# nijaru/sy

Hardware: AMD Instinct MI355X
Metric: GiB/s device-resident delta signature+match, 4 KiB blocks; % HBM-read peak (higher is better)
Workload: dtype u8

## Files before the change

### sy_amd/csrc/sydelta_kernels.hip

```cpp
#include "sydelta_device.hpp"
#include "sydelta_internal.hpp"
#include "sydelta_zstdbatch.hpp"

#include <hipcub/hipcub.hpp>

#include <algorithm>
#include <chrono>
#include <mutex>

namespace sydelta {

#include "sydelta_kcommon.hpp"


__global__ __launch_bounds__(256) void k_sig_fast(const uint8_t* __restrict__ buf, uint64_t nfull, uint32_t bs,
                                                  uint32_t* __restrict__ weak, uint64_t* __restrict__ strong) {
    const uint32_t lane = threadIdx.x & 63;
    const uint64_t blk = ((((uint64_t)blockIdx.x * blockDim.x + threadIdx.x) >> 6) << 2) + (lane >> 4);
    if ((blk & ~3ull) >= nfull) return;
    const bool live = blk < nfull;
    uint32_t wk;
    uint64_t st;
    row_hash(buf + (live ? blk : (nfull - 1)) * (uint64_t)bs, bs, wk, st);
    if ((lane & 15) == 0 && live) {
// ... 962 lines not shown
                si = cur->seg_id;
                if (p < cur->pos_end) {
                    slot = table_find(cur->keys, cur->bmask, ew);
                    fslot = (uint32_t)cur->slot_off;
                }
                rp = (uint32_t)(p - cur->pos_begin);
            } else {
                const uint32_t t = t_begin + (ex >> 14);
                si = seg_of_tile(a, t);
                const ScanSeg S = a.segs[si];
                const uint64_t p = S.pos_begin + (uint64_t)(t - S.tile_base) * kTile2 + (ex & (kTile2 - 1));
                if (p < S.pos_end) {
                    const FileIx F = a.files[S.file];
                    slot = table_find(a.keys + F.slot_off, F.bmask, ew);
                    fslot = (uint32_t)F.slot_off;
                }
                rp = (uint32_t)(p - S.pos_begin);
            }
        }
        const bool hit = slot >= 0;
        const uint64_t m = __ballot(hit);
        if (!m) continue;
        const uint32_t cnt = __popcll(m);
        weak_hits += cnt;
        if (nwq + cnt > (uint32_t)kWQ2) {
            lds_fence();
            verify3<kRowVerify>(a, wq, nwq, rows, tile_start, cur);
            nwq = 0;
        }
        if (hit) wq[nwq + __popcll(m & ((1ull << lane) - 1))] = make_uint4(si, rp, fslot + (uint32_t)slot, 0);
        nwq += cnt;
    }
    lds_fence();
    if (tw) { const unsigned long long t1 = __builtin_amdgcn_s_memtime(); t_lk += t1 - t0; t0 = t1; }
    verify3<kRowVerify>(a, wq, nwq, rows, tile_start, cur);
    lds_fence();
    if (tw) {
        t_vf += __builtin_amdgcn_s_memtime() - t0;
        atomicAdd(&a.counters[8], t_lk);
        atomicAdd(&a.counters[9], t_vf);
    }
}

template <bool kLdsFilter, int kWgPerCu = kLdsFilter ? 3 : 4, bool kRowVerify = false>
__global__ __launch_bounds__(kT2, kWgPerCu) void k_scan_lds(ScanArgs a, uint32_t per, uint32_t lds_fwords) {
    constexpr bool kTileFlush = !kLdsFilter;
    extern __shared__ __attribute__((aligned(16))) unsigned char smem[];
    const uint32_t n = a.n;
    const Lds2 L = lds2_layout(n, kLdsFilter ? lds_fwords : 0u);
    uint32_t* rows = (uint32_t*)smem;
    uint32_t* PS = (uint32_t*)(smem + L.ps);
    uint32_t* PV = (uint32_t*)(smem + L.pv);
    uint64_t* PJ = (uint64_t*)(smem + L.pj);
    uint32_t* ntab = (uint32_t*)(smem + L.ntab);
    uint32_t* lfilt = (uint32_t*)(smem + L.filt);
    const uint32_t tid = threadIdx.x;
    const uint32_t lane = tid & 63, wid = tid >> 6;
    uint4* wq = (uint4*)(smem + L.q) + (size_t)wid * kWQ2;
    uint2* fq = a.gfq + ((size_t)blockIdx.x * (kT2 / 64) + wid) * kGFQ;
    __shared__ uint32_t red_s[kT2 / 64], red_v[kT2 / 64];
    __shared__ uint64_t red_j[kT2 / 64];

    const uint32_t t_begin = blockIdx.x * per;
    const uint32_t t_end = min(a.ntiles, t_begin + per);
    if (t_begin >= t_end) return;
    const uint32_t nch = L.nch;

    for (uint32_t i = tid; i < 256; i += kT2) ntab[i] = kMod - 1 - (a.nm * i) % kMod;
    const uint32_t sh = n & 3;
    const uint32_t rel0 = tid * kR2;
    unsigned long long passes = 0, weak_hits = 0;
    uint32_t nfq = 0;
    uint32_t cur_file = 0xFFFFFFFFu;
    uint32_t fwshift = 0;
    const uint32_t* gfilt = a.filt;
    SegCtx sc;

    unsigned long long tm[4] = {0, 0, 0, 0};
    unsigned long long tprev = a.timing ? __builtin_amdgcn_s_memtime() : 0;
#define PHASE_MARK(k)                                                  \
    if (a.timing) {                                                    \
        const unsigned long long tnow = __builtin_amdgcn_s_memtime(); \
        tm[k] += tnow - tprev;                                         \
        tprev = tnow;                                                  \
    }
    uint32_t si = 0;
#pragma unroll 1
    for (uint32_t tile = t_begin; tile < t_end; ++tile) {
        if (tile == t_begin || (si + 1 < a.nsegs && a.segs[si + 1].tile_base <= tile)) {
            uint32_t lo = si, hi = a.nsegs;
            if (tile == t_begin) lo = 0;
            while (hi - lo > 1) {
                const uint32_t mid = (lo + hi) >> 1;
                if (a.segs[mid].tile_base <= tile) lo = mid; else hi = mid;
            }
            si = lo;
            const ScanSeg S = a.segs[si];
            const FileIx F = a.files[S.file];
            sc.base = a.src + S.src;
            sc.pos_begin = S.pos_begin;
            sc.pos_end = S.pos_end;
            sc.keys = a.keys + F.slot_off;
            sc.slot_off = F.slot_off;
            sc.bmask = F.bmask;
            sc.seg_id = si;
            fwshift = F.fwshift;
            gfilt = a.filt + F.filt_off;
            if (kLdsFilter && S.file != cur_file) {
                const uint4* src4 = (const uint4*)gfilt;
                uint4* dst4 = (uint4*)lfilt;
                const uint32_t fwords = 1u << (32 - fwshift);
#pragma unroll 4
                for (uint32_t i = tid; i < fwords / 4; i += kT2) dst4[i] = src4[i];
            }
            cur_file = S.file;
        }
        const uint64_t seg_len = a.segs[si].len;
        const uint64_t tile_start = sc.pos_begin + (uint64_t)(tile - a.segs[si].tile_base) * kTile2;

#pragma unroll 1
        for (uint32_t c = tid; c < nch; c += kT2) {
            uint32_t x[16];
            load_chunk_nt(sc.base, seg_len, tile_start + 64ull * c, x);
            uint32_t S = 0, V = 0;
#pragma unroll
            for (int i = 0; i < 16; ++i) {
                S = udot4(x[i], 0x01010101u, S);
                V = udot4(x[i], offw(i), V);
                rows[c * kRowDw + i] = x[i];
            }
            PS[c] = S;
            PV[c] = V;
        }
        __syncthreads();
        PHASE_MARK(0)

        {
            const uint32_t per_t = (nch + kT2 - 1) / kT2;
            const uint32_t c_lo = min(nch, tid * per_t), c_hi = min(nch, c_lo + per_t);
            uint32_t ts = 0, tv = 0;
            uint64_t tj = 0;
            for (uint32_t c = c_lo; c < c_hi; ++c) { ts += PS[c]; tv += PV[c]; tj += (uint64_t)c * PS[c]; }
            uint32_t is = ts, iv = tv;
            uint64_t ij = tj;
#pragma unroll
            for (int m = 1; m < 64; m <<= 1) {
                const uint32_t os = (uint32_t)__shfl_up((int)is, m, 64);
                const uint32_t ov = (uint32_t)__shfl_up((int)iv, m, 64);
                const uint32_t ojl = (uint32_t)__shfl_up((int)(uint32_t)ij, m, 64);
                const uint32_t ojh = (uint32_t)__shfl_up((int)(uint32_t)(ij >> 32), m, 64);
                if (lane >= (uint32_t)m) { is += os; iv += ov; ij += ((uint64_t)ojh << 32) | ojl; }
            }
            if (lane == 63) { red_s[wid] = is; red_v[wid] = iv; red_j[wid] = ij; }
            __syncthreads();
            uint32_t bs_ = 0, bv_ = 0;
            uint64_t bj_ = 0;
            for (uint32_t w = 0; w < wid; ++w) { bs_ += red_s[w]; bv_ += red_v[w]; bj_ += red_j[w]; }
            uint32_t es = bs_ + is - ts, ev = bv_ + iv - tv;
            uint64_t ej = bj_ + ij - tj;
            for (uint32_t c = c_lo; c < c_hi; ++c) {
                const uint32_t s0 = PS[c], v0 = PV[c];
                PS[c] = es; PV[c] = ev; PJ[c] = ej;
                es += s0; ev += v0; ej += (uint64_t)c * s0;
            }
            if (tid == kT2 - 1) { PS[nch] = bs_ + is; PV[nch] = bv_ + iv; PJ[nch] = bj_ + ij; }
            __syncthreads();
        }

        uint32_t am, bm;
        {
            const uint32_t c0 = tid, m = n >> 6, rem = n & 63;
            const uint64_t dS = PS[c0 + m] - PS[c0];
            const uint64_t dV = PV[c0 + m] - PV[c0];
            const uint64_t dJ = PJ[c0 + m] - PJ[c0];
            uint64_t A = dS;
            uint64_t B = (uint64_t)n * dS - 64ull * (dJ - (uint64_t)c0 * dS) - dV;
            for (uint32_t r = 0; r < rem; ++r) {
                const uint32_t xr = (rows[(c0 + m) * kRowDw + (r >> 2)] >> (8 * (r & 3))) & 0xFF;
                A += xr;
                B += (uint64_t)(rem - r) * xr;
            }
            am = (uint32_t)((1 + A) % kMod);
            bm = (uint32_t)((n + B) % kMod);
        }
        PHASE_MARK(1)

        const uint32_t qtile = (tile - t_begin) << 14;
#pragma unroll 1
        for (uint32_t g = 0; g < (uint32_t)kR2; g += kB2) {
            if (nfq > (uint32_t)(kGFQ - 64 * kB2)) {
                passes += nfq;
                drain3<kRowVerify>(a, fq, nfq, wq, t_begin, weak_hits, kTileFlush ? rows : nullptr, tile_start,
                       kTileFlush ? &sc : nullptr);
                nfq = 0;
            }
            uint32_t xo[4], xi[4];
#pragma unroll
            for (int j = 0; j < 4; ++j) xo[j] = rows[tid * kRowDw + (g >> 2) + j];
            {
                const uint32_t d0 = (rel0 + g + n) >> 2;
                uint32_t dw[5];
#pragma unroll
                for (int j = 0; j < 5; ++j) {
                    const uint32_t d = d0 + j;
                    dw[j] = rows[(d >> 4) * kRowDw + (d & 15)];
                }
#pragma unroll
                for (int j = 0; j < 4; ++j) xi[j] = __builtin_amdgcn_alignbyte(dw[j + 1], dw[j], sh);
            }
            uint32_t ct[kB2];
#pragma unroll
            for (int t = 0; t < kB2; ++t) ct[t] = ntab[(xo[t >> 2] >> (8 * (t & 3))) & 0xFF];
            uint32_t wv[kB2], fh[kB2], fw[kB2];
#pragma unroll
            for (int t = 0; t < kB2; ++t) {
                const uint32_t out = (xo[t >> 2] >> (8 * (t & 3))) & 0xFF;
                const uint32_t in = (xi[t >> 2] >> (8 * (t & 3))) & 0xFF;
                wv[t] = (bm << 16) | am;
                const ProbeHash h = probe_hash(am, bm);
                fh[t] = h.q;
                fw[t] = kLdsFilter ? lfilt[h.r >> fwshift] : gfilt[h.r >> fwshift];
                uint32_t u = am + in - out;
                u = min(u, u + kMod);
                am = min(u, u - kMod);
                uint32_t v = bm + am + ct[t];
                v = min(v, v - kMod);
                bm = min(v, v - kMod);
            }
#pragma unroll
            for (int t = 0; t < kB2; ++t) {
                const bool pass = filt_pass(fw[t], fh[t]);
                const uint64_t mk = __ballot(pass);
                if (mk) {
                    if (pass) fq[nfq + __popcll(mk & ((1ull << lane) - 1))] = make_uint2(qtile | (rel0 + g + t), wv[t]);
                    nfq += __popcll(mk);
                }
            }
        }
        PHASE_MARK(2)
        if (kTileFlush && nfq) {
            passes += nfq;
            drain3<kRowVerify>(a, fq, nfq, wq, t_begin, weak_hits, rows, tile_start, &sc);
            nfq = 0;
        }
        __syncthreads();
        PHASE_MARK(3)
    }
    passes += nfq;
    drain3<kRowVerify>(a, fq, nfq, wq, t_begin, weak_hits);
#undef PHASE_MARK
    if (lane == 0 && passes) atomicAdd(&a.counters[2], passes);
    if (lane == 0 && weak_hits) atomicAdd(&a.counters[1], weak_hits);
    if (a.timing && tid == 0)
        for (int k = 0; k < 4; ++k) atomicAdd(&a.counters[4 + k], tm[k]);
}

constexpr int kB3 = 8;
constexpr uint32_t kMaxN3 = 4096;
constexpr uint32_t kMulti = 0x80000000u;

__device__ __forceinline__ bool fat_find_k(const uint32_t* __restrict__ keys, const uint4* __restrict__ fat,
                                           uint32_t bmask, uint32_t w, uint4& rec) {
    uint32_t b = bucket_hash(w) & bmask;
    for (;;) {
        const uint4 k = *(const uint4*)(keys + 4 * (size_t)b);
        const int j = k.x == w ? 0 : k.y == w ? 1 : k.z == w ? 2 : k.w == w ? 3 : -1;
        if (j >= 0) {
            rec = fat[4 * (size_t)b + j];
            return true;
        }
        if (k.w == kEmptyKey) return false;
        b = (b + 1) & bmask;
    }
}


struct L1Batch {
    uint32_t w2[kB3], hq[kB3], wv[kB3];
};

__device__ __forceinline__ void load16_nt(const uint8_t* src, uint64_t len, uint64_t c0, uint32_t x[4]) {
    if (c0 + 16 <= len) {
        const uint4* q = (const uint4*)(src + c0);
        x[0] = __builtin_nontemporal_load(&q->x);
        x[1] = __builtin_nontemporal_load(&q->y);
        x[2] = __builtin_nontemporal_load(&q->z);
        x[3] = __builtin_nontemporal_load(&q->w);
    } else {
#pragma unroll
        for (int i = 0; i < 4; ++i) {
            uint32_t v = 0;
            for (int b = 0; b < 4; ++b) {
                const uint64_t p = c0 + 4 * i + b;
                if (p < len) v |= (uint32_t)src[p] << (8 * b);
            }
            x[i] = v;
        }
    }
}

constexpr int kTR = 512;
constexpr int kWTR = 4096;
constexpr int kNBR = 64 / kB3;
static_assert(kMaxN3 == 4096 && kWTR % kMaxN3 == 0, "k_scan_r: a lane's in row is row l of the next wave tile");

struct LdsR {
    uint32_t l1, ntab, kt, ctr, total;
};
__host__ __device__ constexpr LdsR ldsr_layout() {
    LdsR L{};
    uint32_t o = 0;
    L.l1 = o; o += kL1WordsR * 4;
    L.ntab = o; o += 256 * 4;
    L.kt = o; o += 48 * 8;
    L.ctr = o; o += 16;
    L.total = o;
    return L;
}
static_assert(ldsr_layout().total <= 160 * 1024 - 256, "k_scan_r's LDS");

constexpr int kKtW = 0, kKtLast = 24, kKtInit = 32, kKtMerge = 40, kKtWords = 48;
typedef uint32_t v16u32 __attribute__((ext_vector_type(16)));

__device__ __forceinline__ uint64_t dpp64_ctrl_shr4(uint64_t v) {
    return ((uint64_t)dpp32<0x114>((uint32_t)(v >> 32)) << 32) | dpp32<0x114>((uint32_t)v);
}
__device__ __forceinline__ uint64_t dpp64_ctrl_shl4(uint64_t v) {
    return ((uint64_t)dpp32<0x104>((uint32_t)(v >> 32)) << 32) | dpp32<0x104>((uint32_t)v);
}
template <int kCtrl>
__device__ __forceinline__ uint64_t dpp64(uint64_t v) {
    return ((uint64_t)dpp32<kCtrl>((uint32_t)(v >> 32)) << 32) | dpp32<kCtrl>((uint32_t)v);
}

__device__ __forceinline__ uint64_t wave_strong_regs(const uint32_t (&xo)[16], const uint32_t (&xi)[16], uint32_t o,
                                                  const uint64_t* kt) {
    const uint32_t lane = threadIdx.x & 63;
    o = __builtin_amdgcn_readfirstlane(o);
    const uint32_t lp = o >> 6, c = o & 63, q = c >> 2, sh = c & 3;
    v16u32 S0, S1;
#pragma unroll
    for (int r = 0; r < 16; ++r) {
        S0[r] = lane >= lp ? xo[r] : xi[r];
        S1[r] = lane > lp ? xo[r] : xi[r];
    }
    const int addrA = (int)(((lp + lane) & 63) << 2), addrB = (int)(((lp + lane + 1) & 63) << 2);
    uint32_t raw[17];
#pragma unroll
    for (int j = 0; j < 17; ++j) {
        const uint32_t r = q + j;
        const uint32_t v = r < 16 ? S0[r & 15] : S1[r & 15];
        raw[j] = (uint32_t)__builtin_amdgcn_ds_bpermute(r < 16 ? addrA : addrB, (int)v);
    }
    const uint32_t kb = lane == 63 ? (uint32_t)kKtLast : (lane & 15);
    uint64_t cc[8];
#pragma unroll
    for (int i = 0; i < 8; ++i) cc[i] = 0;
#pragma unroll
    for (int i = 0; i < 8; ++i) {
        const uint32_t w0 = __builtin_amdgcn_alignbyte(raw[2 * i + 1], raw[2 * i], sh);
        const uint32_t w1 = __builtin_amdgcn_alignbyte(raw[2 * i + 2], raw[2 * i + 1], sh);
        const uint64_t v = (uint64_t)w0 | ((uint64_t)w1 << 32);
        const uint64_t dk = v ^ kt[kb + i];
        cc[i ^ 1] += v;
        cc[i] += mul32x32(dk);
    }
    uint64_t f;
    const bool b3 = lane & 8, b2 = lane & 4, b1 = lane & 2;
    uint64_t d[4], e[2];
#pragma unroll
    for (int k = 0; k < 4; ++k) {
        const uint64_t send = b3 ? cc[k] : cc[4 + k], keep = b3 ? cc[4 + k] : cc[k];
        d[k] = keep + dpp64<kDppRowRor8>(send);
    }
#pragma unroll
    for (int k = 0; k < 2; ++k) {
        const uint64_t send = b2 ? d[k] : d[2 + k], keep = b2 ? d[2 + k] : d[k];
        const uint64_t from_lo = dpp64_ctrl_shr4(send), from_hi = dpp64_ctrl_shl4(send);
        e[k] = keep + (b2 ? from_lo : from_hi);
    }
    {
        const uint64_t send = b1 ? e[0] : e[1], keep = b1 ? e[1] : e[0];
        f = keep + dpp64<kDppQuadXor2>(send);
    }
    f += dpp64<kDppQuadXor1>(f);
    const uint64_t p1 = shfl64(f, (int)((lane + 16) & 63));
    const uint64_t p2 = shfl64(f, (int)((lane + 32) & 63));
    const uint64_t p3 = shfl64(f, (int)((lane + 48) & 63));
    const uint32_t ai = (lane >> 1) & 7;
    const uint64_t skey = kt[kKtW + 16 + ai];
    uint64_t acc = kt[kKtInit + ai] + f;
    acc = scramble1(acc, skey) + p1;
    acc = scramble1(acc, skey) + p2;
    acc = scramble1(acc, skey) + p3;
    const uint64_t z = acc ^ kt[kKtMerge + ai];
    const uint64_t zp = dpp64<kDppQuadXor2>(z);
    uint64_t m = (lane & 3) == 0 ? fold64(z, zp) : 0ull;
    m += dpp64<kDppRowRor4>(m);
    m += dpp64<kDppRowRor8>(m);
    const uint64_t h = xxh3_aval((uint64_t)4096 * P64_1 + m);
    return ((uint64_t)__builtin_amdgcn_readlane((int)(uint32_t)(h >> 32), 0) << 32) |
           (uint32_t)__builtin_amdgcn_readlane((int)(uint32_t)h, 0);
}

constexpr uint32_t kHStage = 256;
constexpr uint32_t kDStage = 64;

struct WaveOut {
    uint4* h;
    WDef* d;
    uint32_t nh;
    uint32_t nd;
};

__device__ __forceinline__ WaveOut wave_out(const ScanArgs& a, uint64_t gwave) {
    WaveOut o;
    o.h = a.hstage + gwave * kHStage;
    o.d = a.dstage ? a.dstage + gwave * kDStage : nullptr;
    o.nh = 0;
    o.nd = 0;
    return o;
}

__device__ __forceinline__ void flush_hits(const ScanArgs& a, WaveOut& o) {
    if (!o.nh) return;
    const uint32_t lane = threadIdx.x & 63;
    __threadfence_block();
    unsigned long long k0 = 0;
    if (lane == 0) k0 = atomicAdd(&a.counters[0], (unsigned long long)o.nh);
    k0 = shfl64(k0, 0);
    for (uint32_t i = lane; i < o.nh; i += 64) {
        const volatile uint4* g = o.h + i;
        const uint32_t lo = g->x, hi = g->y, blk = g->z;
        const unsigned long long k = k0 + i;
        if (k < a.out_cap) {
            a.hit_key[k] = ((uint64_t)hi << 32) | lo;
            a.hit_val[k] = blk;
        }
    }
    o.nh = 0;
}

__device__ __forceinline__ void stage_hits(const ScanArgs& a, WaveOut& o, bool v, uint64_t key, uint32_t blk) {
    const uint64_t m = __ballot(v);
    if (!m) return;
    const uint32_t c = __popcll(m);
    if (o.nh + c > kHStage) flush_hits(a, o);
    const uint32_t lane = threadIdx.x & 63;
    if (v) o.h[o.nh + __popcll(m & ((1ull << lane) - 1))] = make_uint4((uint32_t)key, (uint32_t)(key >> 32), blk, 0);
    o.nh += c;
}

__device__ __forceinline__ uint32_t verify_def(const ScanArgs& a, const WDef& d) {
    uint64_t st;
    if (a.n > 240) {
        uint32_t wk;
        wave_hash_long(a.src + d.at, a.n, wk, st);
    } else {
        st = 0;
        if ((threadIdx.x & 63) == 0) st = xxh3_short(a.src + d.at, a.n);
        st = shfl64(st, 0);
    }
    if (!(d.cand & kMulti)) return st == d.strong ? d.cand : kNoBlock;
    return first_strong_match(a.order, a.cstrong, a.start[d.cand & ~kMulti], a.cnt[d.cand & ~kMulti], st);
}

__device__ __forceinline__ void flush_defs(const ScanArgs& a, WaveOut& o) {
    if (!o.nd) return;
    const uint32_t lane = threadIdx.x & 63;
    __threadfence_block();
    unsigned long long k0 = 0;
    if (lane == 0) k0 = atomicAdd(&a.counters[10], (unsigned long long)o.nd);
    k0 = shfl64(k0, 0);
    for (uint32_t i = lane; i < o.nd; i += 64) {
        const unsigned long long k = k0 + i;
        if (k < a.wdef_cap) {
            const volatile uint64_t* g = (const volatile uint64_t*)(o.d + i);
            WDef d;
            d.at = g[0];
            d.key = g[1];
            const uint64_t cp = g[2];
            d.cand = (uint32_t)cp;
            d.pad = 0;
            d.strong = g[3];
            a.wdef[k] = d;
        }
    }
    if (k0 + o.nd > a.wdef_cap) {
        const uint32_t first = k0 >= a.wdef_cap ? 0u : (uint32_t)(a.wdef_cap - k0);
        for (uint32_t i = first; i < o.nd; ++i) {
            const volatile uint64_t* g = (const volatile uint64_t*)(o.d + i);
            WDef d;
            d.at = g[0];
            d.key = g[1];
            d.cand = (uint32_t)g[2];
            d.pad = 0;
            d.strong = g[3];
            const uint32_t best = verify_def(a, d);
            stage_hits(a, o, lane == 0 && best != kNoBlock, d.key, best);
        }
    }
    o.nd = 0;
}

__device__ __forceinline__ void stage_defs(const ScanArgs& a, WaveOut& o, bool v, const WDef& d) {
    const uint64_t m = __ballot(v);
    if (!m) return;
    const uint32_t c = __popcll(m);
    if (o.nd + c > kDStage) flush_defs(a, o);
    const uint32_t lane = threadIdx.x & 63;
    if (v) o.d[o.nd + __popcll(m & ((1ull << lane) - 1))] = d;
    o.nd += c;
}

template <bool kSmall = false>
__device__ __forceinline__ void drain_regs(const ScanArgs& a, const uint2* recs, uint32_t nr, uint32_t tile_rel,
                                           const uint32_t (&xo)[16], const uint32_t (&xi)[16], const uint64_t* kt,
                                           unsigned long long& weak_hits, uint64_t run_start, const SegCtx& cur,
                                           WaveOut& o) {
    const uint32_t lane = threadIdx.x & 63;
    __threadfence_block();
    for (uint32_t base = 0; base < nr; base += 64) {
        const uint32_t i = base + lane;
        bool hit = false;
        uint4 rec = make_uint4(0, 0, 0, 0);
        uint32_t pos = 0;
        if (i < nr) {
            const volatile uint2* g = recs + i;
            pos = g->x;
            const uint32_t w = g->y;
            if (run_start + pos < cur.pos_end) {
                if (kSmall) {
                    const int64_t sl = table_find(cur.keys, cur.bmask, w);
                    hit = sl >= 0;
                    rec.y = kMulti | (uint32_t)(cur.slot_off + (uint64_t)(sl < 0 ? 0 : sl));
                } else {
                    hit = fat_find_k(cur.keys, cur.fat, cur.bmask, w, rec);
                }
            }
        }
        uint64_t m = __ballot(hit);
        weak_hits += __popcll(m);
        uint32_t best_mine = kNoBlock;
        while (m) {
            const int h = __builtin_ctzll(m);
            m &= m - 1;
            const uint32_t hp = __builtin_amdgcn_readlane((int)pos, h);
            const uint32_t hy = __builtin_amdgcn_readlane((int)rec.y, h);
            const uint64_t hs = ((uint64_t)(uint32_t)__builtin_amdgcn_readlane((int)rec.w, h) << 32) |
                                (uint32_t)__builtin_amdgcn_readlane((int)rec.z, h);
            const uint64_t st = wave_strong_regs(xo, xi, hp - tile_rel, kt);
            uint32_t best = kNoBlock;
            if (!(hy & kMulti)) {
                if (st == hs) best = hy;
            } else {
                best = first_strong_match(a.order, a.cstrong, a.start[hy & ~kMulti], a.cnt[hy & ~kMulti], st);
            }
            if ((int)lane == h) best_mine = best;
        }
        stage_hits(a, o, best_mine != kNoBlock,
                   ((uint64_t)cur.seg_id << kSegShift) | (uint64_t)(run_start + pos - cur.pos_begin), best_mine);
    }
}

template <bool kRib, int kWaves, bool kSmall = false>
__global__ __launch_bounds__(kWaves * 64, 1) void k_scan_r(ScanArgs a, uint32_t per, uint32_t small_words) {
    extern __shared__ __attribute__((aligned(16))) unsigned char smem[];
    constexpr LdsR L = ldsr_layout();
    constexpr uint32_t kT = kWaves * 64;
    const uint32_t n = a.n;
    const uint32_t* l1 = (const uint32_t*)(smem + L.l1);
    uint32_t* ntab = (uint32_t*)(smem + L.ntab);
    const uint32_t tid = threadIdx.x;
    const uint32_t lane = tid & 63, wid = tid >> 6;
    uint32_t* ctr = (uint32_t*)(smem + L.ctr);
    const uint32_t gwave = blockIdx.x * kWaves + wid;
    uint2* rec = a.rrec + (size_t)gwave * kWTR;
    uint32_t* fslot = (uint32_t*)(smem + L.l1) + (size_t)wid * small_words;
    uint32_t slot_file = 0xFFFFFFFFu;
    WaveOut wo = wave_out(a, gwave);

    const uint32_t t_begin = blockIdx.x * per;
    const uint32_t t_end = min(a.ntiles, t_begin + per);
    if (t_begin >= t_end) return;
    if (!kSmall) {
        const uint4* g = (const uint4*)a.l1;
        uint4* d = (uint4*)(smem + L.l1);
#pragma unroll 4
        for (uint32_t i = tid; i < kL1WordsR / 4; i += kT) d[i] = g[i];
    }
    for (uint32_t i = tid; i < 256; i += kT) ntab[i] = kMod - 1 - (a.nm * i) % kMod;
    uint64_t* kt = (uint64_t*)(smem + L.kt);
    if (tid < 48)
        kt[tid] = tid < 24 ? c_tab.w[tid] : tid < 32 ? c_tab.last[tid - 24] : tid < 40 ? c_tab.init[tid - 32]
                                                                                       : c_tab.merge[tid - 40];
    if (tid == 0) *ctr = 0;
    __syncthreads();

    unsigned long long passes = 0, weak_hits = 0;
    uint32_t nrec = 0, si_hint = 0;
    const uint64_t below = (1ull << lane) - 1;
#pragma unroll 1
    for (;;) {
        uint32_t c = 0;
        if (lane == 0) c = atomicAdd(ctr, 1u);
        c = __builtin_amdgcn_readfirstlane(c);
        const uint32_t t0 = t_begin + 2 * c;
        if (t0 >= t_end) break;
        const uint32_t tz = min(t_end, t0 + 2);
#pragma unroll 1
        for (uint32_t t = t0; t < tz;) {
            uint32_t lo = si_hint, hi = a.nsegs;
            while (hi - lo > 1) {
                const uint32_t mid = (lo + hi) >> 1;
                if (a.segs[mid].tile_base <= t) lo = mid; else hi = mid;
            }
            const uint32_t si = lo;
            si_hint = si;
            const ScanSeg S = a.segs[si];
            const FileIx F = a.files[S.file];
            SegCtx sc;
            sc.base = a.src + S.src;
            sc.pos_begin = S.pos_begin;
            sc.keys = a.keys + F.slot_off;
            sc.fat = a.fat + F.slot_off;
            sc.slot_off = F.slot_off;
            sc.bmask = F.bmask;
            sc.seg_id = si;
            sc.fwshift = F.fwshift;
            sc.filt = a.filt + F.filt_off;
            sc.fwords = 1u << (32 - F.fwshift);
            const uint32_t span = (t + 1 < tz && !(si + 1 < a.nsegs && a.segs[si + 1].tile_base <= t + 1)) ? 2u : 1u;
            const uint64_t run_start = S.pos_begin + (uint64_t)(t - S.tile_base) * kTile2;
            sc.pos_end = min(S.pos_end, run_start + (uint64_t)span * kTile2);
            const uint64_t seg_len = S.len;
            const uint32_t nwt = span * (kTile2 / kWTR);
            t += span;

            const uint64_t fptr = (uint64_t)(uintptr_t)sc.filt;
            const uint32_t fp_lo = __builtin_amdgcn_readfirstlane((uint32_t)fptr);
            const uint32_t fp_hi = __builtin_amdgcn_readfirstlane((uint32_t)(fptr >> 32));
            const __amdgpu_buffer_rsrc_t frsrc = __builtin_amdgcn_make_buffer_rsrc(
                (void*)(uintptr_t)(((uint64_t)fp_hi << 32) | fp_lo), (short)0,
                (int)__builtin_amdgcn_readfirstlane(sc.fwords * 4), 0x00020000);
            const uint32_t fwshift = __builtin_amdgcn_readfirstlane(sc.fwshift);
            if (kSmall && S.file != slot_file) {
                slot_file = S.file;
                lds_fence();
                const uint4* g = (const uint4*)sc.filt;
                uint4* d = (uint4*)fslot;
                for (uint32_t i = lane; i < sc.fwords / 4; i += 64) d[i] = g[i];
                lds_fence();
            }

            uint32_t xo[16], xi[16], xn[16];
            load_chunk_nt(sc.base, seg_len, run_start + 64ull * lane, xo);
            load_chunk_nt(sc.base, seg_len, run_start + n + 64ull * lane, xi);
#pragma unroll 1
            for (uint32_t k = 0; k < nwt; ++k) {
                const uint64_t P = run_start + (uint64_t)k * kWTR;
                const uint32_t rel0 = k * kWTR + lane * 64;
                uint32_t am, bm;
                {
                    uint32_t Sx[2], Vx[2], Jx[2], TS[2], TV[2], TJ[2];
#pragma unroll
                    for (int j = 0; j < 2; ++j) {
                        uint32_t s = 0, v = 0;
#pragma unroll
                        for (int i = 0; i < 16; ++i) {
                            const uint32_t d = j ? xi[i] : xo[i];
                            s = udot4(d, 0x01010101u, s);
                            v = udot4(d, offw(i), v);
                        }
                        Sx[j] = wave_scan_excl(s, TS[j]);
                        Vx[j] = wave_scan_excl(v, TV[j]);
                        Jx[j] = wave_scan_excl((uint32_t)(64 * j + lane) * s, TJ[j]);
                    }
                    const uint64_t dS = TS[0] + Sx[1] - Sx[0];
                    const uint64_t dV = TV[0] + Vx[1] - Vx[0];
                    const uint64_t dJ = TJ[0] + Jx[1] - Jx[0];
                    const uint32_t A = (uint32_t)dS;
                    const uint32_t B = (uint32_t)((uint64_t)n * dS - 64ull * (dJ - (uint64_t)lane * dS) - dV);
                    am = (1 + A) % kMod;
                    bm = (n + B) % kMod;
                }
                auto compute = [&](const int g, L1Batch& Bt) {
                    const uint32_t xo0 = xo[g >> 2], xo1 = xo[(g >> 2) + 1];
                    const uint32_t xi0 = xi[g >> 2], xi1 = xi[(g >> 2) + 1];
                    uint32_t ct[kB3], rr[kB3], w1[kB3], w1b[kB3], bo[kB3];
#pragma unroll
                    for (int t2 = 0; t2 < kB3; ++t2) ct[t2] = ntab[((t2 < 4 ? xo0 : xo1) >> (8 * (t2 & 3))) & 0xFF];
#pragma unroll
                    for (int t2 = 0; t2 < kB3; ++t2) {
                        const uint32_t out = ((t2 < 4 ? xo0 : xo1) >> (8 * (t2 & 3))) & 0xFF;
                        const uint32_t in = ((t2 < 4 ? xi0 : xi1) >> (8 * (t2 & 3))) & 0xFF;
                        __builtin_assume(am < kMod);
                        __builtin_assume(bm < kMod);
                        Bt.wv[t2] = (bm << 16) | am;
                        const ProbeHash h = probe_hash(am, bm);
                        Bt.hq[t2] = h.q;
                        rr[t2] = h.r;
                        if (kSmall) {
                            Bt.w2[t2] = fslot[h.r >> fwshift];
                        } else if (kRib) {
                            bo[t2] = rib_bit(h.q, h.r);
                            w1[t2] = l1[bo[t2] >> 5];
                            w1b[t2] = l1[(bo[t2] >> 5) + 1];
                        } else {
                            w1[t2] = l1[l1r_word(h.q)];
                        }
                        const uint32_t u = am + in + (kMod - out);
                        am = min(u, min(u - kMod, u - 2 * kMod));
                        const uint32_t v = bm + am + ct[t2];
                        bm = min(v, min(v - kMod, v - 2 * kMod));
                    }
#pragma unroll
                    for (int t2 = 0; t2 < kB3 && !kSmall; ++t2) {
                        uint32_t p1;
                        if (kRib) {
                            const uint32_t win = __builtin_amdgcn_alignbit(w1b[t2], w1[t2], bo[t2]);
                            p1 = ~__builtin_popcount(win & rib_coef(Bt.hq[t2], rr[t2])) & 1u;
                        } else {
                            p1 = l1_test(w1[t2], Bt.hq[t2]);
                        }
                        Bt.w2[t2] = __builtin_amdgcn_raw_buffer_load_b32(frsrc, (int)(((rr[t2] >> fwshift) << 2) | (p1 - 1u)),
                                                                         0, 0);
                    }
                };
                auto finish = [&](const int g, L1Batch& Bt) {
                    uint32_t pbits = 0;
#pragma unroll
                    for (int t2 = 0; t2 < kB3; ++t2) pbits |= filt_bit(Bt.w2[t2], Bt.hq[t2]) << t2;
                    asm volatile("" : "+v"(pbits));
                    if (!__ballot(pbits != 0)) return;
#pragma unroll
                    for (int t2 = 0; t2 < kB3; ++t2) {
                        const uint64_t mk = __ballot((pbits >> t2) & 1);
                        if (!mk) continue;
                        if ((pbits >> t2) & 1) rec[nrec + __popcll(mk & below)] = make_uint2(rel0 + g + t2, Bt.wv[t2]);
                        nrec += __popcll(mk);
                    }
                };
                const uint32_t tile_rec = nrec;
                L1Batch b0, b1;
                compute(0, b0);
                compute(8, b1);
#pragma unroll
                for (int bi = 0; bi < kNBR; ++bi) {
                    L1Batch& Bt = (bi & 1) ? b1 : b0;
                    finish(kB3 * bi, Bt);
                    if (bi + 2 < kNBR) compute(kB3 * (bi + 2), Bt);
                    if (bi == 2 && k + 1 < nwt)
                        load_chunk_nt(sc.base, seg_len, P + n + kWTR + 64ull * lane, xn);
                }
                passes += nrec - tile_rec;
                if (nrec > tile_rec)
                    drain_regs<kSmall>(a, rec + tile_rec, nrec - tile_rec, k * kWTR, xo, xi, kt, weak_hits, run_start, sc,
                                       wo);
                nrec = tile_rec;
#pragma unroll
                for (int i = 0; i < 16; ++i) {
                    xo[i] = xi[i];
                    xi[i] = xn[i];
                }
            }
        }
    }
    flush_hits(a, wo);
    if (lane == 0 && passes) atomicAdd(&a.counters[2], passes);
    if (lane == 0 && weak_hits) atomicAdd(&a.counters[1], weak_hits);
}


__device__ __forceinline__ void load64_u(const uint8_t* src, uint64_t len, uint64_t q, uint32_t x[16]) {
    const uint32_t sh = (uint32_t)q & 15u;
    if (!sh) {
        load_chunk(src, len, q, x);
        return;
    }
    const uint64_t qa = q - sh;
    const uint4* g = (const uint4*)(src + qa);
    uint32_t d[20];
    if (qa + 80 <= len) {
#pragma unroll
        for (int i = 0; i < 5; ++i) {
            const uint4 v = g[i];
            d[4 * i] = v.x; d[4 * i + 1] = v.y; d[4 * i + 2] = v.z; d[4 * i + 3] = v.w;
        }
    } else {
#pragma unroll
        for (int i = 0; i < 5; ++i) {
            uint4 v = make_uint4(0, 0, 0, 0);
            if (qa + 16 * i < len) v = g[i];
            d[4 * i] = v.x; d[4 * i + 1] = v.y; d[4 * i + 2] = v.z; d[4 * i + 3] = v.w;
        }
#pragma unroll
        for (int i = 0; i < 20; ++i) {
            const uint64_t o = qa + 4 * i;
            d[i] &= o >= len ? 0u : (o + 4 <= len ? 0xFFFFFFFFu : (0xFFFFFFFFu >> (8 * (o + 4 - len))));
        }
    }
    const uint32_t ds = sh >> 2, bs = sh & 3;
    uint32_t e[17];
#pragma unroll
    for (int i = 0; i < 17; ++i) e[i] = ds == 0 ? d[i] : ds == 1 ? d[i + 1] : ds == 2 ? d[i + 2] : d[i + 3];
#pragma unroll
    for (int i = 0; i < 16; ++i) x[i] = __builtin_amdgcn_alignbyte(e[i + 1], e[i], bs);
}

__device__ __forceinline__ void window_at(const uint8_t* src, uint64_t len, uint64_t P, uint32_t n, uint32_t& am,
                                          uint32_t& bm) {
    const uint32_t lane = threadIdx.x & 63;
    uint64_t s = 0, t = 0;
    for (uint32_t c = 64 * lane; c < n; c += 64 * 64) {
        uint32_t x[16];
        load64_u(src, len, P + c, x);
        uint32_t cs = 0, cv = 0;
#pragma unroll
        for (int i = 0; i < 16; ++i) {
            const uint32_t j = c + 4 * i;
            const uint32_t keep = j >= n ? 0u : (j + 4 <= n ? 0xFFFFFFFFu : (0xFFFFFFFFu >> (8 * (j + 4 - n))));
            const uint32_t v = x[i] & keep;
            cs = udot4(v, 0x01010101u, cs);
            cv = udot4(v, offw(i), cv);
        }
        s += cs;
        t += (uint64_t)c * cs + cv;
    }
    s = wave_sum64(s);
    t = wave_sum64(t);
    am = (uint32_t)((1 + s) % kMod);
    bm = (uint32_t)((n + (uint64_t)n * s - t) % kMod);
}

__device__ __forceinline__ void drain_g(const ScanArgs& a, const uint2* recs, uint32_t nr, unsigned long long& weak_hits,
                                        uint64_t run_start, const SegCtx& cur, WaveOut& o) {
    const uint32_t lane = threadIdx.x & 63;
    __threadfence_block();
    for (uint32_t base = 0; base < nr; base += 64) {
        const uint32_t i = base + lane;
        bool hit = false;
        uint4 rec = make_uint4(0, 0, 0, 0);
        uint32_t pos = 0;
        if (i < nr) {
            const volatile uint2* g = recs + i;
            pos = g->x;
            const uint32_t w = g->y;
            if (run_start + pos < cur.pos_end) hit = fat_find_k(cur.keys, cur.fat, cur.bmask, w, rec);
        }
        const uint64_t m = __ballot(hit);
        if (!m) continue;
        weak_hits += __popcll(m);
        const uint64_t p = run_start + pos;
        WDef d;
        d.at = (uint64_t)(cur.base - a.src) + p;
        d.key = ((uint64_t)cur.seg_id << kSegShift) | (p - cur.pos_begin);
        d.cand = rec.y;
        d.pad = 0;
        d.strong = ((uint64_t)rec.w << 32) | rec.z;
        stage_defs(a, o, hit, d);
    }
}

__device__ __forceinline__ void drain_gs(const ScanArgs& a, const uint2* recs, uint32_t nr,
                                         unsigned long long& weak_hits, uint64_t run_start, const SegCtx& cur,
                                         WaveOut& o) {
    const uint32_t lane = threadIdx.x & 63;
    __threadfence_block();
    for (uint32_t base = 0; base < nr; base += 64) {
        const uint32_t i = base + lane;
        bool hit = false;
        uint32_t pos = 0, gslot = 0;
        if (i < nr) {
            const volatile uint2* g = recs + i;
            pos = g->x;
            const uint32_t w = g->y;
            if (run_start + pos < cur.pos_end) {
                const int64_t sl = table_find(cur.keys, cur.bmask, w);
                hit = sl >= 0;
                gslot = (uint32_t)(cur.slot_off + (uint64_t)(sl < 0 ? 0 : sl));
            }
        }
        const uint64_t m = __ballot(hit);
        if (!m) continue;
        weak_hits += __popcll(m);
        const uint64_t p = run_start + pos;
        WDef d;
        d.at = (uint64_t)(cur.base - a.src) + p;
        d.key = ((uint64_t)cur.seg_id << kSegShift) | (p - cur.pos_begin);
        d.cand = kMulti | gslot;
        d.pad = 0;
        d.strong = 0;
        stage_defs(a, o, hit, d);
    }
}

struct LdsG {
    uint32_t l1, ntab, ctr, total;
};
__host__ __device__ constexpr LdsG ldsg_layout(uint32_t small_words = 0) {
    LdsG L{};
    uint32_t o = 0;
    L.l1 = o; o += small_words ? (kTR / 64) * small_words * 4 : kL1WordsR * 4;
    L.ntab = o; o += 256 * 4;
    L.ctr = o; o += 16;
    L.total = o;
    return L;
}
static_assert(ldsg_layout().total <= 160 * 1024 - 256, "k_scan_g's LDS");

template <bool kRib, bool kSmall>
__global__ __launch_bounds__(kTR, 2) void k_scan_g(ScanArgs a, uint32_t per, uint32_t rt, uint32_t small_words) {
    extern __shared__ __attribute__((aligned(16))) unsigned char smem[];
    const LdsG L = ldsg_layout(kSmall ? small_words : 0u);
    const uint32_t n = a.n;
    const uint32_t* l1 = (const uint32_t*)(smem + L.l1);
    uint32_t* ntab = (uint32_t*)(smem + L.ntab);
    const uint32_t tid = threadIdx.x;
    const uint32_t lane = tid & 63, wid = tid >> 6;
    uint32_t* ctr = (uint32_t*)(smem + L.ctr);
    const uint32_t gwave = blockIdx.x * (kTR / 64) + wid;
    uint2* rec = a.rrec + (size_t)gwave * kWTR;
    WaveOut wo = wave_out(a, gwave);
    uint32_t* fslot = (uint32_t*)(smem + L.l1) + (size_t)wid * small_words;

    const uint32_t t_begin = blockIdx.x * per;
    const uint32_t t_end = min(a.ntiles, t_begin + per);
    if (t_begin >= t_end) return;
    if (!kSmall) {
        const uint4* g = (const uint4*)a.l1;
        uint4* d = (uint4*)(smem + L.l1);
#pragma unroll 4
        for (uint32_t i = tid; i < kL1WordsR / 4; i += kTR) d[i] = g[i];
    }
    for (uint32_t i = tid; i < 256; i += kTR) ntab[i] = kMod - 1 - (a.nm * i) % kMod;
    if (tid == 0) *ctr = 0;
    __syncthreads();

    unsigned long long passes = 0, weak_hits = 0;
    uint32_t nrec = 0, si_hint = 0, slot_file = 0xFFFFFFFFu;
    const uint64_t below = (1ull << lane) - 1;
#pragma unroll 1
    for (;;) {
        uint32_t c = 0;
        if (lane == 0) c = atomicAdd(ctr, 1u);
        c = __builtin_amdgcn_readfirstlane(c);
        const uint32_t t0 = t_begin + rt * c;
        if (t0 >= t_end) break;
        const uint32_t tz = min(t_end, t0 + rt);
#pragma unroll 1
        for (uint32_t t = t0; t < tz;) {
            uint32_t lo = si_hint, hi = a.nsegs;
            while (hi - lo > 1) {
                const uint32_t mid = (lo + hi) >> 1;
                if (a.segs[mid].tile_base <= t) lo = mid; else hi = mid;
            }
            const uint32_t si = lo;
            si_hint = si;
            const ScanSeg S = a.segs[si];
            const FileIx F = a.files[S.file];
            SegCtx sc;
            sc.base = a.src + S.src;
            sc.pos_begin = S.pos_begin;
            sc.keys = a.keys + F.slot_off;
            sc.fat = a.fat + F.slot_off;
            sc.slot_off = F.slot_off;
            sc.bmask = F.bmask;
            sc.seg_id = si;
            sc.fwshift = F.fwshift;
            sc.filt = a.filt + F.filt_off;
            sc.fwords = 1u << (32 - F.fwshift);
            const uint32_t seg_tend = si + 1 < a.nsegs ? a.segs[si + 1].tile_base : a.ntiles;
            const uint32_t span = min(tz, seg_tend) - t;
            const uint64_t run_start = S.pos_begin + (uint64_t)(t - S.tile_base) * kTile2;
            sc.pos_end = min(S.pos_end, run_start + (uint64_t)span * kTile2);
            const uint64_t seg_len = S.len;
            const uint32_t nwt = (uint32_t)((sc.pos_end - run_start + kWTR - 1) / kWTR);
            t += span;

            const uint64_t fptr = (uint64_t)(uintptr_t)sc.filt;
            const uint32_t fp_lo = __builtin_amdgcn_readfirstlane((uint32_t)fptr);
            const uint32_t fp_hi = __builtin_amdgcn_readfirstlane((uint32_t)(fptr >> 32));
            const __amdgpu_buffer_rsrc_t frsrc = __builtin_amdgcn_make_buffer_rsrc(
                (void*)(uintptr_t)(((uint64_t)fp_hi << 32) | fp_lo), (short)0,
                (int)__builtin_amdgcn_readfirstlane(sc.fwords * 4), 0x00020000);
            const uint32_t fwshift = __builtin_amdgcn_readfirstlane(sc.fwshift);
            if (kSmall && S.file != slot_file) {
                slot_file = S.file;
                lds_fence();
                const uint4* g = (const uint4*)sc.filt;
                uint4* d = (uint4*)fslot;
                for (uint32_t i = lane; i < sc.fwords / 4; i += 64) d[i] = g[i];
                lds_fence();
            }

            uint32_t A0, B0;
            window_at(sc.base, seg_len, run_start, n, A0, B0);
            uint32_t xo[16], xi[16], no_[16], ni_[16];
            load_chunk_nt(sc.base, seg_len, run_start + 64ull * lane, xo);
            load64_u(sc.base, seg_len, run_start + n + 64ull * lane, xi);
#pragma unroll 1
            for (uint32_t k = 0; k < nwt; ++k) {
                const uint64_t P = run_start + (uint64_t)k * kWTR;
                const uint32_t rel0 = k * kWTR + lane * 64;
                uint32_t am, bm;
                {
                    uint32_t so = 0, vo = 0, si_ = 0, vi = 0;
#pragma unroll
                    for (int i = 0; i < 16; ++i) {
                        so = udot4(xo[i], 0x01010101u, so);
                        vo = udot4(xo[i], offw(i), vo);
                        si_ = udot4(xi[i], 0x01010101u, si_);
                        vi = udot4(xi[i], offw(i), vi);
                    }
                    uint32_t tot;
                    const uint32_t Ox = wave_scan_excl(so, tot), Ix = wave_scan_excl(si_, tot);
                    const uint32_t ROx = wave_scan_excl(lane * so, tot), RIx = wave_scan_excl(lane * si_, tot);
                    const uint32_t VOx = wave_scan_excl(vo, tot), VIx = wave_scan_excl(vi, tot);
                    const uint64_t d = 64ull * lane;
                    const uint64_t pin = 64ull * ((uint64_t)lane * Ix - RIx) - VIx;
                    const uint64_t pout = 64ull * ((uint64_t)lane * Ox - ROx) - VOx;
                    am = (uint32_t)(((uint64_t)A0 + Ix + 16ull * kMod - Ox) % kMod);
                    const uint64_t bpos = (uint64_t)B0 + d * (A0 + kMod - 1) + pin;
                    const uint64_t bneg = (pout + (uint64_t)a.nm * Ox) % kMod;
                    bm = (uint32_t)((bpos % kMod + kMod - bneg) % kMod);
                }
                auto compute = [&](const int g, L1Batch& Bt) {
                    const uint32_t xo0 = xo[g >> 2], xo1 = xo[(g >> 2) + 1];
                    const uint32_t xi0 = xi[g >> 2], xi1 = xi[(g >> 2) + 1];
                    uint32_t ct[kB3], rr[kB3], w1[kB3], w1b[kB3], bo[kB3];
#pragma unroll
                    for (int t2 = 0; t2 < kB3; ++t2) ct[t2] = ntab[((t2 < 4 ? xo0 : xo1) >> (8 * (t2 & 3))) & 0xFF];
#pragma unroll
                    for (int t2 = 0; t2 < kB3; ++t2) {
                        const uint32_t out = ((t2 < 4 ? xo0 : xo1) >> (8 * (t2 & 3))) & 0xFF;
                        const uint32_t in = ((t2 < 4 ? xi0 : xi1) >> (8 * (t2 & 3))) & 0xFF;
                        __builtin_assume(am < kMod);
                        __builtin_assume(bm < kMod);
                        Bt.wv[t2] = (bm << 16) | am;
                        const ProbeHash h = probe_hash(am, bm);
                        Bt.hq[t2] = h.q;
                        rr[t2] = h.r;
                        if (kSmall) {
                            Bt.w2[t2] = fslot[h.r >> fwshift];
                        } else if (kRib) {
                            bo[t2] = rib_bit(h.q, h.r);
                            w1[t2] = l1[bo[t2] >> 5];
                            w1b[t2] = l1[(bo[t2] >> 5) + 1];
                        } else {
                            w1[t2] = l1[l1r_word(h.q)];
                        }
                        const uint32_t u = am + in + (kMod - out);
                        am = min(u, min(u - kMod, u - 2 * kMod));
                        const uint32_t v = bm + am + ct[t2];
                        bm = min(v, min(v - kMod, v - 2 * kMod));
                    }
#pragma unroll
                    for (int t2 = 0; t2 < kB3 && !kSmall; ++t2) {
                        uint32_t p1;
                        if (kRib) {
                            const uint32_t win = __builtin_amdgcn_alignbit(w1b[t2], w1[t2], bo[t2]);
                            p1 = ~__builtin_popcount(win & rib_coef(Bt.hq[t2], rr[t2])) & 1u;
// ... 2405 lines not shown
```

Measured before the change: 720.5.

## Resolve fat-table lookups cooperatively with four lanes per record in drain

In the non-small path, drain_regs now assigns four lanes to each record, and each lane loads one slot of the 4-wide fat bucket. Probing is resolved with wave ballots, and the matching slot's data is shuffled back via ds_bpermute, handling 32 records per round in two interleaved groups. The aim is to replace serial per-lane probing of a bucket's slots with parallel, coalesced slot loads and to overlap two lookups. The change also uses mbcnt for the prefix count, makes wid wave-uniform, and resets nrec per tile. The cost is fewer records per lane per pass plus extra cross-lane shuffles.

```diff
diff --git a/sy_amd/csrc/sydelta_kernels.hip b/sy_amd/csrc/sydelta_kernels.hip
--- a/sy_amd/csrc/sydelta_kernels.hip
+++ b/sy_amd/csrc/sydelta_kernels.hip
@@ -1288,6 +1288,7 @@
 constexpr int kTR = 512;
 constexpr int kWTR = 4096;
 constexpr int kNBR = 64 / kB3;
+constexpr int kDrainGroup = 32;
 static_assert(kMaxN3 == 4096 && kWTR % kMaxN3 == 0, "k_scan_r: a lane's in row is row l of the next wave tile");
 
 struct LdsR {
@@ -1304,6 +1305,7 @@
     return L;
 }
 static_assert(ldsr_layout().total <= 160 * 1024 - 256, "k_scan_r's LDS");
+static_assert(kDrainGroup == 32, "drain_regs: two rounds of 64 / 4 records");
 
 constexpr int kKtW = 0, kKtLast = 24, kKtInit = 32, kKtMerge = 40, kKtWords = 48;
 typedef uint32_t v16u32 __attribute__((ext_vector_type(16)));
@@ -1499,6 +1501,15 @@
     o.nd += c;
 }
 
+struct QuadLook {
+    uint4 s;
+    uint32_t pos;
+    uint32_t w;
+    uint32_t b;
+    bool look;
+    bool hit;
+};
+
 template <bool kSmall = false>
 __device__ __forceinline__ void drain_regs(const ScanArgs& a, const uint2* recs, uint32_t nr, uint32_t tile_rel,
                                            const uint32_t (&xo)[16], const uint32_t (&xi)[16], const uint64_t* kt,
@@ -1506,25 +1517,14 @@
                                            WaveOut& o) {
     const uint32_t lane = threadIdx.x & 63;
     __threadfence_block();
-    for (uint32_t base = 0; base < nr; base += 64) {
-        const uint32_t i = base + lane;
-        bool hit = false;
-        uint4 rec = make_uint4(0, 0, 0, 0);
-        uint32_t pos = 0;
-        if (i < nr) {
-            const volatile uint2* g = recs + i;
-            pos = g->x;
-            const uint32_t w = g->y;
-            if (run_start + pos < cur.pos_end) {
-                if (kSmall) {
-                    const int64_t sl = table_find(cur.keys, cur.bmask, w);
-                    hit = sl >= 0;
-                    rec.y = kMulti | (uint32_t)(cur.slot_off + (uint64_t)(sl < 0 ? 0 : sl));
-                } else {
-                    hit = fat_find_k(cur.keys, cur.fat, cur.bmask, w, rec);
-                }
-            }
-        }
+    auto rec_at = [&](uint32_t i) -> uint2 {
+        const volatile uint2* g = recs + i;
+        uint2 r;
+        r.x = g->x;
+        r.y = g->y;
+        return r;
+    };
+    auto verify = [&](bool hit, uint32_t pos, const uint4& rec) {
         uint64_t m = __ballot(hit);
         weak_hits += __popcll(m);
         uint32_t best_mine = kNoBlock;
@@ -1546,6 +1546,78 @@
         }
         stage_hits(a, o, best_mine != kNoBlock,
                    ((uint64_t)cur.seg_id << kSegShift) | (uint64_t)(run_start + pos - cur.pos_begin), best_mine);
+    };
+    if (kSmall) {
+        for (uint32_t base = 0; base < nr; base += 64) {
+            const uint32_t i = base + lane;
+            bool hit = false;
+            uint4 rec = make_uint4(0, 0, 0, 0);
+            uint32_t pos = 0;
+            if (i < nr) {
+                const uint2 r = rec_at(i);
+                pos = r.x;
+                if (run_start + pos < cur.pos_end) {
+                    const int64_t sl = table_find(cur.keys, cur.bmask, r.y);
+                    hit = sl >= 0;
+                    rec.y = kMulti | (uint32_t)(cur.slot_off + (uint64_t)(sl < 0 ? 0 : sl));
+                }
+            }
+            verify(hit, pos, rec);
+        }
+        return;
+    }
+    const uint32_t slot = lane & 3, quad0 = lane & ~3u;
+    auto issue = [&](uint32_t base) {
+        QuadLook q;
+        q.s = make_uint4(0, 0, 0, 0);
+        q.pos = q.w = 0;
+        q.b = lane;
+        q.look = q.hit = false;
+        const uint32_t i = base + (lane >> 2);
+        if (i < nr) {
+            const uint2 r = rec_at(i);
+            q.pos = r.x;
+            q.w = r.y;
+            if (run_start + q.pos < cur.pos_end) {
+                q.look = true;
+                q.b = bucket_hash(q.w) & cur.bmask;
+                q.s = cur.fat[4 * (size_t)q.b + slot];
+            }
+        }
+        return q;
+    };
+    auto resolve = [&](QuadLook& q) {
+        while (__ballot(q.look)) {
+            const uint32_t found = (uint32_t)(__ballot(q.look && q.s.x == q.w) >> quad0) & 0xFu;
+            const bool open = (__ballot(q.look && q.s.x == kEmptyKey) >> (quad0 + 3)) & 1;
+            if (q.look) {
+                if (found) {
+                    q.hit = true;
+                    q.b = quad0 + (uint32_t)__builtin_ctz(found);
+                    q.look = false;
+                } else if (open) {
+                    q.b = lane;
+                    q.look = false;
+                } else {
+                    q.b = (q.b + 1) & cur.bmask;
+                    q.s = cur.fat[4 * (size_t)q.b + slot];
+                }
+            }
+        }
+    };
+    for (uint32_t base = 0; base < nr; base += kDrainGroup) {
+        QuadLook q0 = issue(base), q1 = issue(base + kDrainGroup / 2);
+        resolve(q0);
+        resolve(q1);
+        const int f0 = (int)(q0.b << 2), f1 = (int)(q1.b << 2);
+        uint4 rec = make_uint4(0, 0, 0, 0);
+        const uint32_t y0 = __builtin_amdgcn_ds_bpermute(f0, (int)q0.s.y), y1 = __builtin_amdgcn_ds_bpermute(f1, (int)q1.s.y);
+        const uint32_t z0 = __builtin_amdgcn_ds_bpermute(f0, (int)q0.s.z), z1 = __builtin_amdgcn_ds_bpermute(f1, (int)q1.s.z);
+        const uint32_t w0 = __builtin_amdgcn_ds_bpermute(f0, (int)q0.s.w), w1 = __builtin_amdgcn_ds_bpermute(f1, (int)q1.s.w);
+        rec.y = slot ? y1 : y0;
+        rec.z = slot ? z1 : z0;
+        rec.w = slot ? w1 : w0;
+        verify(slot == 0 ? q0.hit : slot == 1 && q1.hit, slot ? q1.pos : q0.pos, rec);
     }
 }
 
@@ -1558,7 +1630,7 @@
     const uint32_t* l1 = (const uint32_t*)(smem + L.l1);
     uint32_t* ntab = (uint32_t*)(smem + L.ntab);
     const uint32_t tid = threadIdx.x;
-    const uint32_t lane = tid & 63, wid = tid >> 6;
+    const uint32_t lane = tid & 63, wid = __builtin_amdgcn_readfirstlane(tid >> 6);
     uint32_t* ctr = (uint32_t*)(smem + L.ctr);
     const uint32_t gwave = blockIdx.x * kWaves + wid;
     uint2* rec = a.rrec + (size_t)gwave * kWTR;
@@ -1585,7 +1657,6 @@
 
     unsigned long long passes = 0, weak_hits = 0;
     uint32_t nrec = 0, si_hint = 0;
-    const uint64_t below = (1ull << lane) - 1;
 #pragma unroll 1
     for (;;) {
         uint32_t c = 0;
@@ -1723,11 +1794,14 @@
                     for (int t2 = 0; t2 < kB3; ++t2) {
                         const uint64_t mk = __ballot((pbits >> t2) & 1);
                         if (!mk) continue;
-                        if ((pbits >> t2) & 1) rec[nrec + __popcll(mk & below)] = make_uint2(rel0 + g + t2, Bt.wv[t2]);
+                        if ((pbits >> t2) & 1) {
+                            const uint32_t at = __builtin_amdgcn_mbcnt_hi((uint32_t)(mk >> 32), __builtin_amdgcn_mbcnt_lo((uint32_t)mk, 0u));
+                            rec[nrec + at] = make_uint2(rel0 + g + t2, Bt.wv[t2]);
+                        }
                         nrec += __popcll(mk);
                     }
                 };
-                const uint32_t tile_rec = nrec;
+                nrec = 0;
                 L1Batch b0, b1;
                 compute(0, b0);
                 compute(8, b1);
@@ -1739,11 +1813,8 @@
                     if (bi == 2 && k + 1 < nwt)
                         load_chunk_nt(sc.base, seg_len, P + n + kWTR + 64ull * lane, xn);
                 }
-                passes += nrec - tile_rec;
-                if (nrec > tile_rec)
-                    drain_regs<kSmall>(a, rec + tile_rec, nrec - tile_rec, k * kWTR, xo, xi, kt, weak_hits, run_start, sc,
-                                       wo);
-                nrec = tile_rec;
+                passes += nrec;
+                if (nrec) drain_regs<kSmall>(a, rec, nrec, k * kWTR, xo, xi, kt, weak_hits, run_start, sc, wo);
 #pragma unroll
                 for (int i = 0; i < 16; ++i) {
                     xo[i] = xi[i];
```

Measured after the change: 729.1, median of 6. +1.2%, better.
